# foollh/PicoPose

Measured on AMD Instinct MI355X. Metric: image-crops/sec (224x224, 162 templates), higher is better.
Workload: dtype f32 tensors; networks: f32 operands split into 2 f16 terms (22 bits) on f16 MFMA with f32 accumulate; stage-1 contraction: f16 MFMA operands, f32 accumulate, exact f32 re-evaluation of near-ties; PnP f64

## Files before the change

include/picopose_hip.h:

```cpp
#ifndef PICOPOSE_HIP_H
#define PICOPOSE_HIP_H

#include <stddef.h>
#include <stdint.h>

#ifdef __cplusplus
extern "C" {
#endif

#define PP_OK 0
#define PP_EINVAL (-1)
#define PP_EWORKSPACE (-2)
#define PP_ELAUNCH (-3)

#define PP_MATCH_EXACT 0
#define PP_MATCH_FAST 1

const char* pp_strerror(int code);
int pp_version(void);

int pp_prof_enable(int max_records);
int pp_prof_collect(float* out_ms, int max_out, int* count);
int pp_prof_gemm_enable(int max_records);
int pp_prof_gemm_collect(double* ms, double* flops, int* launches);
// ... 161 lines not shown
int pp_transpose_batched(const float* in, long long in_batch_stride, int B, int R, int C, float* out,
                         long long out_batch_stride, int ld_out, int col_off, void* stream);
int pp_assemble_tokens(const float* patches, const float* cls_token, const float* pos, int B, int T, int C,
                       float* tokens, void* stream);
int pp_normalize_rows(const float* x, int rows, int n, float eps, float* y, void* stream);

int pp_resize_bilinear_nhwc(const float* in, int B, int H, int W, int C, int Ho, int Wo, float mul,
                            float* out, void* stream);
int pp_resize_bilinear_nhwc_hl(const float* in, int B, int H, int W, int C, int Ho, int Wo, float mul, void* out_hl,
                               void* stream);
int pp_warp_nhwc(const float* feat, int feat_batch, const float* flow, int B, int H, int W, int C, int ld_flow,
                 float* out, int ld_out, void* stream);
int pp_warp_nhwc_hl(const float* feat, int feat_batch, const float* flow, int B, int H, int W, int C, int ld_flow,
                    void* out_hl, int ld_h, void* stream);
int pp_avgpool2_nhwc(const float* in, int B, int H, int W, int C, float* out, void* stream);
int pp_gather_rows(const float* src, const long long* index, long long n_src_rows, long long row_floats, int n, float* dst,
                   void* stream);
int pp_bank_rows_to_tokens(const float* bank, long long n_bank_rows, int C, int P, const long long* index, int n, float* tokens, int ld,
                           int T, int skip, void* stream);
int pp_patch_operand(const float* bank, long long n_bank_rows, const long long* index, int n, const float* front, int n_front, int H, int W,
                     void* out, int terms, void* stream);
int pp_flow_operand(const float* flow, int ld_flow, long long rows, void* out8, int terms, void* stream);

int pp_crop_resize_normalize(const unsigned char* image, int H, int W, const unsigned char* mask, int y1, int y2, int x1,
                             int x2, int S, int rgb_mask_flag, const double* mean3, const double* std3, float* out_rgb,
                             float* out_mask, void* stream);
int pp_depth_points_nearest(const float* depth_m, int H, int W, int y1, int y2, int x1, int x2, int P, float fx, float fy,
                            float cx, float cy, float* out_pts, void* stream);
int pp_corr_lookup_nhwc(const float* f1, int ld_f1, const float* f2_l0, const float* f2_l1, const float* f2_l2,
                        int f2_batch, const float* flow, int B, int H, int W, int C, int levels, int radius,
                        int ld_flow, float* out, int ld_out, void* stream);
int pp_corr_lookup_nhwc_ex(const float* f1, int ld_f1, const float* f2_l0, const float* f2_l1, const float* f2_l2,
                           int f2_batch, const float* flow, int B, int H, int W, int C, int levels, int radius,
                           int ld_flow, int prec, float* out, int ld_out, void* stream);

int pp_conv_narrow_hl(const void* x_hl, int ld_x, int B, int H, int W, int C, const float* weight, const float* bias, int ksize,
                      int n_out, const float* residual, float* out, void* stream);
int pp_conv_narrow_f32(const float* x, int ld_x, int B, int H, int W, int C, const float* weight, const float* bias, int ksize,
                       int n_out, const float* residual, float* out, void* stream);

int pp_winograd_input_f32(const float* x, int ld_x, long long batch_stride, int B, int H, int W, int C, int relu, float* U, void* stream);
int pp_winograd_weight_f32(const float* w, int Cout, int Cin, int ldw, float* V, void* stream);
int pp_winograd_output_f32(const float* Y, int B, int H, int W, int Cout, const float* bias, int act, const float* residual,
                           const float* residual2, float* out, int ldc, void* stream);

int pp_winograd4_input_hl(const void* x_hl, int ld_x, long long batch_stride, int B, int H, int W, int C, int relu, void* U_hl, long long P_pad,
                          void* stream);
int pp_winograd4_weight_f32(const float* w, int Cout, int Cin, int ldw, float* V, void* stream);
int pp_winograd4_output(const float* Y, int ld_y, int B, int H, int W, int Cout, const float* bias, int act, const float* residual,
                        const float* residual2, float* out, int ldc, void* out_hl, int ld_h, int c_relu, long long P_pad, void* stream);

int pp_winograd4_chain(const float* Y, int ld_y, int B, int H, int W, int C, const float* bias, int act, int c_relu, void* U_hl, long long P_pad,
                       void* stream);

int pp_winograd_chain_f32(const float* Y, int B, int H, int W, int C, const float* bias, int act, int relu_next, float* U, void* stream);

int pp_set_saturation_word(unsigned int* word);

int pp_saturation_take(unsigned int* word, unsigned int* slot, void* stream);


int pp_corr_lookup_nhwc_hl(const void* f1_hl, int ld_f1, const void* f2_hl_l0, const void* f2_hl_l1, const void* f2_hl_l2,
                           int f2_batch, const float* flow, int B, int H, int W, int C, int levels, int radius, int ld_flow,
                           float* out, int ld_out, void* stream);
int pp_corr_lookup_nhwc_hl_op(const void* f1_hl, int ld_f1, const void* f2_hl_l0, const void* f2_hl_l1, const void* f2_hl_l2,
                              int f2_batch, const float* flow, int B, int H, int W, int C, int levels, int radius, int ld_flow,
                              float* out, int ld_out, void* out_hl, int ld_out_h, void* stream);
int pp_avgpool2_hl(const float* in, int B, int H, int W, int C, float* out, void* out_hl, void* stream);

int pp_pnp_ransac(const float* tar_pts_2d, const float* src_pts_3d, const float* K, const float* tem_pose,
                  const int64_t* tar_pts, const int64_t* src_pts, int P, int H, int W, int N, int iterations,
                  float reproj_threshold, double* rot, double* tvec, double* inlier_ratio, int32_t* success,
                  int32_t* num_points, void* stream);

int pp_pnp_ransac_debug(const float* tar_pts_2d, const float* src_pts_3d, const float* K, const float* tem_pose,
                        const int64_t* tar_pts, const int64_t* src_pts, int P, int H, int W, int N, int iterations,
                        float reproj_threshold, double* rot, double* tvec, double* inlier_ratio, int32_t* success,
                        int32_t* num_points, double* refit_branches, void* stream);

int pp_pnp_ransac_refine(const float* tar_pts_2d, const float* src_pts_3d, const float* K, const float* tem_pose,
                         const int64_t* tar_pts, const int64_t* src_pts, int P, int H, int W, int N, int iterations,
                         float reproj_threshold, int max_iters, double eps, double* rot, double* tvec, double* inlier_ratio,
                         int32_t* success, int32_t* num_points, double* rms_before, double* rms_after, int32_t* lm_iterations,
                         uint8_t* inlier_mask, void* stream);

int pp_pnp_refine_lm(const double* object_points, const double* image_points, const int32_t* count, const double* K,
                     const double* rot_init, const double* tvec_init, int P, int Nmax, int max_iters, double eps, double* rot,
                     double* tvec, double* rms_before, double* rms_after, int32_t* lm_iterations, void* stream);

int pp_rgbd_ransac(const float* tar_pts_2d, const float* src_pts_3d, const float* K, const float* tem_pose,
                   const int64_t* tar_pts, const int64_t* src_pts, int P, int H, int W, int N,
                   const float* depth, int n_images, int dH, int dW, const int32_t* image_index,
                   const float* inlier_dist, int iterations,
                   double* rot, double* tvec, double* inlier_ratio, int32_t* success,
                   int32_t* num_points, int32_t* num_listed, double* rms, uint8_t* inlier_mask, void* stream);

size_t pp_train_keypoints_workspace_bytes(int B);
int pp_train_keypoints(const float* src_mask, const float* tar_mask, int mask_h, int mask_w, const float* src_depth,
                       const float* tar_depth, int depth_h, int depth_w, const float* src_Minv, const float* tar_Minv,
                       const float* src_M, const float* tar_M, const float* src_Kinv, const float* tar_Kinv, const float* src_K,
                       const float* tar_K, const float* T_src2tar, const float* T_tar2src, int B, float* src_pts, float* tar_pts,
                       void* workspace, size_t workspace_bytes, void* stream);
size_t pp_batchnorm_train_workspace_bytes(int rows, int C);
int pp_batchnorm_train(const float* x, const float* gamma, const float* beta, int rows, int C, float eps, float momentum,
                       float* running_mean, float* running_var, int relu, const float* residual, const float* residual2, float* y,
                       void* workspace, size_t workspace_bytes, void* stream);
// ... 236 lines not shown
```

picopose_amd/_lib.py:

```python
import ctypes
import os
import re

from .build import LIB

_HEADER = os.path.join(os.path.dirname(os.path.abspath(__file__)), "..", "include", "picopose_hip.h")

PP_OK = 0
PP_MATCH_EXACT = 0
PP_MATCH_FAST = 1
PP_BANK_F32 = 0
PP_BANK_F16 = 1

_lib = None


class PpGemmDesc(ctypes.Structure):
    _fields_ = [
        ("A", ctypes.c_void_p), ("B", ctypes.c_void_p), ("C", ctypes.c_void_p), ("bias", ctypes.c_void_p),
        ("gamma", ctypes.c_void_p), ("residual", ctypes.c_void_p), ("residual2", ctypes.c_void_p),
        ("M", ctypes.c_int), ("N", ctypes.c_int), ("K", ctypes.c_int),
        ("lda", ctypes.c_int), ("ldb", ctypes.c_int), ("ldc", ctypes.c_int), ("b_kn", ctypes.c_int),
        ("batch0", ctypes.c_int), ("batch1", ctypes.c_int),
        ("a_bs0", ctypes.c_longlong), ("a_bs1", ctypes.c_longlong), ("b_bs0", ctypes.c_longlong),
# ... 40 lines not shown
        if not os.path.exists(LIB):
            raise PicoPoseHipError(
                f"{LIB} not found: build it with `python -m picopose_amd.build` "
                "(hipcc --offload-arch=gfx950). There is no CPU fallback."
            )
        import torch

        L = ctypes.CDLL(LIB)
        c = ctypes
        vp, i32, f32, sz = c.c_void_p, c.c_int, c.c_float, c.c_size_t
        L.pp_strerror.restype = c.c_char_p
        L.pp_strerror.argtypes = [i32]
        L.pp_version.restype = i32
        L.pp_prof_enable.argtypes = [i32]
        L.pp_prof_collect.argtypes = [c.POINTER(f32), i32, c.POINTER(i32)]
        L.pp_prof_gemm_enable.argtypes = [i32]
        L.pp_prof_gemm_collect.argtypes = [c.POINTER(c.c_double), c.POINTER(c.c_double), c.POINTER(i32)]
        L.pp_prof_gemm_records.argtypes = [i32, c.POINTER(i32), c.POINTER(f32), c.POINTER(c.c_double), c.POINTER(i32)]
        L.pp_prof_gemm_records2.argtypes = [i32, c.POINTER(i32), c.POINTER(f32), c.POINTER(c.c_double), c.POINTER(c.c_double), c.POINTER(i32)]
        L.pp_gemm_tune_save.argtypes = [c.c_char_p]
        L.pp_gemm_tune_load.argtypes = [c.c_char_p]
        L.pp_gemm_tune_entries.argtypes = []
        L.pp_gemm_generic_epilogue.argtypes = [i32]
        L.pp_stage1_workspace_bytes.argtypes = [i32, i32, i32, c.POINTER(sz)]
        L.pp_stage1_scores.argtypes = [vp, vp, vp, i32, i32, i32, i32, i32, i32, f32, vp, sz, vp, vp, vp]
        L.pp_stage1_scores_ex.argtypes = [vp, i32, vp, vp, i32, i32, i32, i32, i32, i32, f32, vp, sz, vp, vp, vp]
        L.pp_topk.argtypes = [vp, i32, i32, i32, vp, vp, vp]
        L.pp_stage1_match.argtypes = [vp, vp, vp, i32, i32, i32, i32, i32, i32, i32, f32, vp, sz,
                                      vp, vp, vp, vp, vp]
        L.pp_stage1_match_ex.argtypes = [vp, i32, vp, vp, i32, i32, i32, i32, i32, i32, i32, f32, vp, sz, vp, vp, vp, vp, vp]
        L.pp_stage1_indexed_workspace_bytes.argtypes = [i32, i32, i32, c.POINTER(sz)]
        L.pp_stage1_scores_indexed.argtypes = [vp, i32, vp, i32, vp, vp, i32, i32, i32, i32, i32, i32, f32, vp, sz, vp, vp, vp]
        L.pp_stage1_match_indexed.argtypes = [vp, i32, vp, i32, vp, vp, i32, i32, i32, i32, i32, i32, i32, f32, vp, sz, vp, vp, vp,
                                              vp, vp]
        L.pp_similarity_volume.argtypes = [vp, vp, vp, i32, i32, i32, i32, vp, vp]
        L.pp_calc_pred_Ms.argtypes = [vp, vp, vp, vp, vp, vp, i32, f32, vp, vp]
        L.pp_pose_recovery_2d.argtypes = [vp, vp, vp, vp, vp, vp, i32, vp, vp]
        L.pp_init_correspondences.argtypes = [vp, vp, i32, i32, i32, vp, vp, vp]
        L.pp_stage3_correspondences.argtypes = [vp, vp, i32, i32, i32, f32, vp, vp, vp]
        L.pp_gather_valid.argtypes = [vp, vp, i32, i32, i32, i32, i32, vp, vp, vp]
        L.pp_gemm.argtypes = [c.POINTER(PpGemmDesc), vp]
        L.pp_split_f16x3.argtypes = [vp, c.c_longlong, vp, vp, vp]
        L.pp_split_activation.argtypes = [vp, c.c_longlong, i32, i32, i32, i32, i32, vp, vp]
        L.pp_split_activation_ld.argtypes = [vp, c.c_longlong, i32, i32, i32, i32, i32, vp, i32, vp]
        L.pp_conv_narrow_hl.argtypes = [vp, i32, i32, i32, i32, i32, vp, vp, i32, i32, vp, vp, vp]
        L.pp_conv_narrow_f32.argtypes = [vp, i32, i32, i32, i32, i32, vp, vp, i32, i32, vp, vp, vp]
        L.pp_winograd_input_f32.argtypes = [vp, i32, c.c_longlong, i32, i32, i32, i32, i32, vp, vp]
        L.pp_winograd_weight_f32.argtypes = [vp, i32, i32, i32, vp, vp]
        L.pp_winograd_output_f32.argtypes = [vp, i32, i32, i32, i32, vp, i32, vp, vp, vp, i32, vp]
        L.pp_winograd4_input_hl.argtypes = [vp, i32, c.c_longlong, i32, i32, i32, i32, i32, vp, c.c_longlong, vp]
        L.pp_winograd4_weight_f32.argtypes = [vp, i32, i32, i32, vp, vp]
        L.pp_winograd4_output.argtypes = [vp, i32, i32, i32, i32, i32, vp, i32, vp, vp, vp, i32, vp, i32, i32, c.c_longlong, vp]
        L.pp_winograd4_chain.argtypes = [vp, i32, i32, i32, i32, i32, vp, i32, i32, vp, c.c_longlong, vp]
        L.pp_winograd_chain_f32.argtypes = [vp, i32, i32, i32, i32, vp, i32, i32, vp, vp]
        L.pp_set_saturation_word.argtypes = [vp]
        L.pp_saturation_take.argtypes = [vp, vp, vp]
        L.pp_split_weights_t.argtypes = [vp, c.c_longlong, i32, vp, vp, vp]
        L.pp_split_weights_ws.argtypes = [vp, c.c_longlong, i32, vp, vp, vp, vp]
        L.pp_split_activation_t.argtypes = [vp, c.c_longlong, i32, i32, i32, i32, i32, vp, i32, i32, vp]
        L.pp_hl_patch_columns_t.argtypes = [vp, i32, i32, c.c_longlong, vp, i32, i32, i32, vp]
        L.pp_layernorm_t.argtypes = [vp, vp, vp, i32, i32, f32, vp, vp, i32, vp]
        L.pp_resize_bilinear_nhwc_t.argtypes = [vp, i32, i32, i32, i32, i32, i32, f32, vp, i32, vp]
        L.pp_resize_bilinear_nhwc_dual.argtypes = [vp, i32, i32, i32, i32, i32, i32, f32, vp, vp, i32, vp]
        L.pp_warp_nhwc_t.argtypes = [vp, i32, vp, i32, i32, i32, i32, i32, vp, i32, i32, vp]
        L.pp_attention_t.argtypes = [vp, i32, i32, i32, i32, i32, f32, vp, vp, vp]
        L.pp_sum_slices.argtypes = [vp, i32, i32, i32, vp, i32, vp, vp]
        L.pp_hl_patch_columns.argtypes = [vp, i32, i32, c.c_longlong, vp, i32, i32, vp]
        L.pp_warp_nhwc_hl.argtypes = [vp, i32, vp, i32, i32, i32, i32, i32, vp, i32, vp]
        L.pp_attention.argtypes = [vp, i32, i32, i32, i32, f32, vp, vp]
        L.pp_attention_split.argtypes = [vp, i32, i32, i32, i32, f32, vp, vp, vp]
        L.pp_attention_ex.argtypes = [vp, i32, i32, i32, i32, f32, i32, vp, vp, vp]
        L.pp_attention_hl.argtypes = [vp, i32, i32, i32, i32, f32, vp, vp, vp]
        L.pp_attention_train.argtypes = [vp, i32, i32, i32, i32, f32, vp, vp, vp]
        L.pp_attention_backward.argtypes = [vp, vp, vp, vp, vp, i32, i32, i32, i32, f32, vp, vp, vp]
        L.pp_layernorm.argtypes = [vp, vp, vp, i32, i32, f32, vp, vp]
        L.pp_layernorm_split.argtypes = [vp, vp, vp, i32, i32, f32, vp, vp, vp]
        L.pp_softmax_rows.argtypes = [vp, i32, i32, i32, vp]
        L.pp_groupnorm_nhwc.argtypes = [vp, vp, vp, i32, i32, i32, i32, f32, i32, vp, vp]
        L.pp_transpose_batched.argtypes = [vp, c.c_longlong, i32, i32, i32, vp, c.c_longlong, i32, i32, vp]
        L.pp_assemble_tokens.argtypes = [vp, vp, vp, i32, i32, i32, vp, vp]
        L.pp_normalize_rows.argtypes = [vp, i32, i32, f32, vp, vp]
        L.pp_resize_bilinear_nhwc.argtypes = [vp, i32, i32, i32, i32, i32, i32, f32, vp, vp]
        L.pp_resize_bilinear_nhwc_hl.argtypes = [vp, i32, i32, i32, i32, i32, i32, f32, vp, vp]
        L.pp_warp_nhwc.argtypes = [vp, i32, vp, i32, i32, i32, i32, i32, vp, i32, vp]
        L.pp_avgpool2_nhwc.argtypes = [vp, i32, i32, i32, i32, vp, vp]
        L.pp_gather_rows.argtypes = [vp, vp, c.c_longlong, c.c_longlong, i32, vp, vp]
        L.pp_bank_rows_to_tokens.argtypes = [vp, c.c_longlong, i32, i32, vp, i32, vp, i32, i32, i32, vp]
        L.pp_patch_operand.argtypes = [vp, c.c_longlong, vp, i32, vp, i32, i32, i32, vp, i32, vp]
        L.pp_flow_operand.argtypes = [vp, i32, c.c_longlong, vp, i32, vp]
        L.pp_depth_points_nearest.argtypes = [vp, i32, i32, i32, i32, i32, i32, i32, f32, f32, f32, f32, vp, vp]
        L.pp_crop_resize_normalize.argtypes = [vp, i32, i32, vp, i32, i32, i32, i32, i32, i32, c.POINTER(c.c_double),
                                               c.POINTER(c.c_double), vp, vp, vp]
        L.pp_corr_lookup_nhwc.argtypes = [vp, i32, vp, vp, vp, i32, vp, i32, i32, i32, i32, i32, i32, i32, vp, i32, vp]
        L.pp_corr_lookup_nhwc_ex.argtypes = [vp, i32, vp, vp, vp, i32, vp, i32, i32, i32, i32, i32, i32, i32, i32, vp, i32, vp]
        L.pp_corr_lookup_nhwc_hl.argtypes = [vp, i32, vp, vp, vp, i32, vp, i32, i32, i32, i32, i32, i32, i32, vp, i32, vp]
        L.pp_corr_lookup_nhwc_hl_op.argtypes = [vp, i32, vp, vp, vp, i32, vp, i32, i32, i32, i32, i32, i32, i32, vp, i32, vp, i32, vp]
        L.pp_avgpool2_hl.argtypes = [vp, i32, i32, i32, i32, vp, vp, vp]
        L.pp_pnp_ransac.argtypes = [vp, vp, vp, vp, vp, vp, i32, i32, i32, i32, i32, f32, vp, vp, vp, vp, vp, vp]
        L.pp_pnp_ransac_debug.argtypes = [vp, vp, vp, vp, vp, vp, i32, i32, i32, i32, i32, f32, vp, vp, vp, vp, vp, vp, vp]
        L.pp_pnp_ransac_refine.argtypes = [vp, vp, vp, vp, vp, vp, i32, i32, i32, i32, i32, f32, i32, c.c_double] + [vp] * 10
        L.pp_pnp_refine_lm.argtypes = [vp] * 6 + [i32, i32, i32, c.c_double] + [vp] * 6
        L.pp_rgbd_ransac.argtypes = [vp] * 6 + [i32] * 4 + [vp, i32, i32, i32, vp, vp, i32] + [vp] * 9
        L.pp_train_keypoints_workspace_bytes.restype = sz
        L.pp_train_keypoints_workspace_bytes.argtypes = [i32]
        L.pp_train_keypoints.argtypes = [vp, vp, i32, i32, vp, vp, i32, i32] + [vp] * 10 + [i32, vp, vp, vp, sz, vp]
        L.pp_batchnorm_train_workspace_bytes.restype = sz
# ... 113 lines not shown
```

picopose_amd/csrc/pp_winograd.hip:

```cpp
#include <hip/hip_runtime.h>
#include <stdint.h>
#include "../../include/picopose_hip.h"
#include "pp_common.h"

namespace {

typedef float f4 __attribute__((ext_vector_type(4)));

__device__ __forceinline__ void wino_bt_d_b(const f4 (&d)[4][4], f4 (&u)[4][4]) {
    f4 t[4][4];
#pragma unroll
    for (int c = 0; c < 4; ++c) {
        t[0][c] = d[0][c] - d[2][c];
        t[1][c] = d[1][c] + d[2][c];
        t[2][c] = d[2][c] - d[1][c];
        t[3][c] = d[1][c] - d[3][c];
    }
#pragma unroll
    for (int a = 0; a < 4; ++a) {
        u[a][0] = t[a][0] - t[a][2];
        u[a][1] = t[a][1] + t[a][2];
        u[a][2] = t[a][2] - t[a][1];
        u[a][3] = t[a][1] - t[a][3];
    }
// ... 410 lines not shown
                    wino_split4(x4, hi, lo, top);
#pragma unroll
                    for (int e = 0; e < 4; ++e) f[e] = (float)hi[e] + (float)lo[e];
                    *(f4*)(slot + ((oy * W) + 4 * tx + ox) * CHN_PX + 4 * q) = f;
                }
            }
        }
        if (half >= 1 && live && r >= 2) {
            constexpr int RPG = 6 / NB;
            const int R = r - 2, a0 = NB == 2 ? RPG * (half - 1) : 0;
            f4 t[6][6];
#pragma unroll
            for (int dx = 0; dx < 6; ++dx) {
                f4 d[6];
                const int px = 4 * tx - 1 + dx;
#pragma unroll
                for (int dy = 0; dy < 6; ++dy) {
                    const int g = 4 * R - 1 + dy;
                    const int gc = min(max(g, 0), H - 1), pc = min(max(px, 0), W - 1);
                    f4 v = *(const f4*)(chs + ((gc >> 2) & 3) * SLOT + ((gc & 3) * W + pc) * CHN_PX + 4 * q);
                    if (!(g >= 0 && g < H && px >= 0 && px < W)) v = f4{0.f, 0.f, 0.f, 0.f};
                    d[dy] = v;
                }
                PP_W4_BT(d[0], d[1], d[2], d[3], d[4], d[5], t[0][dx], t[1][dx], t[2][dx], t[3][dx], t[4][dx], t[5][dx])
            }
            const long long p = ((long long)b * th + R) * TW + tx;
            const unsigned uoff = (unsigned)((p * 2 * C + gcol + par * 8) * 2);
#pragma unroll
            for (int ai = 0; ai < RPG; ++ai) {
                f4 u[6];
                if constexpr (NB == 2) {
                    f4 t0 = t[ai][0], t1 = t[ai][1], t2 = t[ai][2], t3 = t[ai][3], t4 = t[ai][4], t5 = t[ai][5];
                    if (a0) {
                        t0 = t[3 + ai][0], t1 = t[3 + ai][1], t2 = t[3 + ai][2];
                        t3 = t[3 + ai][3], t4 = t[3 + ai][4], t5 = t[3 + ai][5];
                    }
                    PP_W4_BT(t0, t1, t2, t3, t4, t5, u[0], u[1], u[2], u[3], u[4], u[5])
                } else {
                    PP_W4_BT(t[ai][0], t[ai][1], t[ai][2], t[ai][3], t[ai][4], t[ai][5], u[0], u[1], u[2], u[3], u[4], u[5])
                }
#pragma unroll
                for (int bb = 0; bb < 6; ++bb) {
                    hf4 hi, lo;
                    wino_split4(u[bb] * (1.f / 64.f), hi, lo, top);
                    __builtin_amdgcn_raw_buffer_store_b128(wino_pair_pack(par, hi, lo), wino_block_rsrc(U, wino_opaque(6 * (a0 + ai) + bb), blk), uoff, 0, PP_WINO_ST_AUX);
                }
            }
        }
        __syncthreads();
    }
    wino_note_sat(!(top < 65504.f), sat);
}

template <int W>
__global__ __launch_bounds__(2 * (W / 2) * 8, 4) void wino2_chain_kernel(const float* __restrict__ Y, int H, int C, long long P, const float* __restrict__ bias,
                                                                       int act, int relu_next, float* __restrict__ U) {
    constexpr int TW = W / 2, NI = TW * 8;
    constexpr int SLOT = 2 * W * CHN_PX;
    extern __shared__ __attribute__((aligned(16))) float chs[];
    const int th = H >> 1, nsl = C >> 5;
    const int b = blockIdx.x / nsl, cs = blockIdx.x - b * nsl;
    const int half = threadIdx.x / NI, it = threadIdx.x - half * NI, tx = it >> 3, q = it & 7;
    const int c = cs * 32 + 4 * q;
    const f4 bv = bias ? *(const f4*)(bias + c) : f4{0.f, 0.f, 0.f, 0.f};
    for (int r = 0; r < th + 2; ++r) {
        if (half == 0 && r < th) {
            const long long p = ((long long)b * th + r) * TW + tx;
            f4 y[4][4];
#pragma unroll
            for (int a = 0; a < 4; ++a)
#pragma unroll
                for (int bb = 0; bb < 4; ++bb) y[a][bb] = *(const f4*)(Y + ((long long)(4 * a + bb) * P + p) * C + c);
            float* slot = chs + (r & 3) * SLOT;
#pragma unroll
            for (int oy = 0; oy < 2; ++oy)
#pragma unroll
                for (int ox = 0; ox < 2; ++ox) {
                    f4 col[4], o;
#pragma unroll
                    for (int bb = 0; bb < 4; ++bb) col[bb] = oy == 0 ? (y[0][bb] + y[1][bb]) + y[2][bb] : (y[1][bb] - y[2][bb]) - y[3][bb];
                    o = ox == 0 ? (col[0] + col[1]) + col[2] : (col[1] - col[2]) - col[3];
#pragma unroll
                    for (int e = 0; e < 4; ++e) {
                        float v = wino_act(o[e] + bv[e], act);
                        o[e] = relu_next ? (v > 0.f ? v : 0.f) : v;
                    }
                    *(f4*)(slot + (oy * W + 2 * tx + ox) * CHN_PX + 4 * q) = o;
                }
        }
        if (half == 1 && r >= 2) {
            const int R = r - 2;
            f4 t[4][4];
#pragma unroll
            for (int dx = 0; dx < 4; ++dx) {
                f4 d[4];
#pragma unroll
                for (int dy = 0; dy < 4; ++dy) {
                    const int g = 2 * R - 1 + dy, px = 2 * tx - 1 + dx;
                    const int gc = min(max(g, 0), H - 1), pc = min(max(px, 0), W - 1);
                    f4 v = *(const f4*)(chs + ((gc >> 1) & 3) * SLOT + ((gc & 1) * W + pc) * CHN_PX + 4 * q);
                    if (!(g >= 0 && g < H && px >= 0 && px < W)) v = f4{0.f, 0.f, 0.f, 0.f};
                    d[dy] = v;
                }
                t[0][dx] = d[0] - d[2];
                t[1][dx] = d[1] + d[2];
                t[2][dx] = d[2] - d[1];
                t[3][dx] = d[1] - d[3];
            }
            const long long p = ((long long)b * th + R) * TW + tx;
#pragma unroll
            for (int a = 0; a < 4; ++a) {
                const f4 u0 = t[a][0] - t[a][2], u1 = t[a][1] + t[a][2], u2 = t[a][2] - t[a][1], u3 = t[a][1] - t[a][3];
                *(f4*)(U + ((long long)(4 * a + 0) * P + p) * C + c) = u0;
                *(f4*)(U + ((long long)(4 * a + 1) * P + p) * C + c) = u1;
                *(f4*)(U + ((long long)(4 * a + 2) * P + p) * C + c) = u2;
                *(f4*)(U + ((long long)(4 * a + 3) * P + p) * C + c) = u3;
            }
        }
        __syncthreads();
    }
}

template <int W>
static int wino2_chain_launch(const float* Y, int B, int H, int C, const float* bias, int act, int relu_next, float* U, hipStream_t st) {
    constexpr int threads = 2 * (W / 2) * 8;
    const size_t lds = (size_t)4 * 2 * W * CHN_PX * sizeof(float);
    static signed char attr[PP_MAX_DEVICES];
    signed char& ok = attr[pp_cur_device()];
    if (ok == 0)
        ok = hipFuncSetAttribute((const void*)wino2_chain_kernel<W>, hipFuncAttributeMaxDynamicSharedMemorySize, (int)lds) == hipSuccess ? 1 : -1;
    if (ok < 0) return PP_ELAUNCH;
    const long long P = (long long)B * (H / 2) * (W / 2);
    hipLaunchKernelGGL(wino2_chain_kernel<W>, dim3((unsigned)(B * (C / 32))), dim3(threads), lds, st, Y, H, C, P, bias, act, relu_next, U);
    return pp_last_launch();
}

template <int W>
static int wino4_chain_launch(const float* Y, int B, int H, int C, const float* bias, int act, int c_relu, void* U, long long Pp, int ldy, hipStream_t st) {
    constexpr int NB = W == 64 ? 2 : 1;
    constexpr int threads = (1 + NB) * ((W / 4) * 8 < 64 ? 64 : (W / 4) * 8);
    const size_t lds = (size_t)4 * 4 * W * CHN_PX * sizeof(float);
    static signed char attr[PP_MAX_DEVICES];
    signed char& ok = attr[pp_cur_device()];
    if (ok == 0)
        ok = hipFuncSetAttribute((const void*)wino4_chain_kernel<W, NB>, hipFuncAttributeMaxDynamicSharedMemorySize, (int)lds) == hipSuccess ? 1 : -1;
    if (ok < 0) return PP_ELAUNCH;
    hipLaunchKernelGGL((wino4_chain_kernel<W, NB>), dim3((unsigned)(B * (C / 32))), dim3(threads), lds, st, Y, H, C, bias, act, c_relu, (_Float16*)U, Pp,
                       ldy, pp_saturation_word());
    return pp_last_launch();
}

static inline int grid8_of(long long n) {
    const long long g = ((n + 255) / 256 + 7) / 8 * 8;
    return (int)g;
}

static inline int grid_of(long long n) {
    const long long g = (n + 255) / 256;
    return (int)(g < 1 ? 1 : (g > 65535 * 8 ? 65535 * 8 : g));
}

}

extern "C" {

int pp_winograd_input_f32(const float* x, int ld_x, long long batch_stride, int B, int H, int W, int C, int relu, float* U, void* stream) {
    if (!x || !U || B <= 0 || H < 2 || W < 2 || (H & 1) || (W & 1) || C <= 0 || (C & 3) || ld_x < C || (ld_x & 3) || (batch_stride & 3)) return PP_EINVAL;
    if (((uintptr_t)x & 15) || ((uintptr_t)U & 15)) return PP_EINVAL;
    const long long total = (long long)B * (H / 2) * (W / 2) * (C / 4);
    hipLaunchKernelGGL(wino_input_kernel, dim3(grid_of(total)), dim3(256), 0, (hipStream_t)stream, x, ld_x, batch_stride, B, H, W, C, relu, U);
    return pp_last_launch();
}

int pp_winograd_weight_f32(const float* w, int Cout, int Cin, int ldw, float* V, void* stream) {
    if (!w || !V || Cout <= 0 || Cin <= 0 || ldw < 9 * Cin) return PP_EINVAL;
    hipLaunchKernelGGL(wino_weight_kernel, dim3(grid_of((long long)Cout * Cin)), dim3(256), 0, (hipStream_t)stream, w, Cout, Cin, ldw, V);
    return pp_last_launch();
}

int pp_winograd_output_f32(const float* Y, int B, int H, int W, int Cout, const float* bias, int act, const float* residual,
                           const float* residual2, float* out, int ldc, void* stream) {
    if (!Y || !out || B <= 0 || H < 2 || W < 2 || (H & 1) || (W & 1) || Cout <= 0 || ldc < Cout) return PP_EINVAL;
    if (act != PP_ACT_NONE && act != PP_ACT_RELU && act != PP_ACT_LEAKY01) return PP_EINVAL;
    const bool vec = (Cout & 3) == 0 && (ldc & 3) == 0 && (((uintptr_t)Y | (uintptr_t)out | (uintptr_t)residual | (uintptr_t)residual2 | (uintptr_t)bias) & 15) == 0;
    const long long total = (long long)B * (H / 2) * (W / 2) * (vec ? Cout / 4 : Cout);
    if (vec)
        hipLaunchKernelGGL(wino_output_kernel<true>, dim3(grid_of(total)), dim3(256), 0, (hipStream_t)stream, Y, B, H, W, Cout, bias, act, residual,
                           residual2, out, ldc);
    else
        hipLaunchKernelGGL(wino_output_kernel<false>, dim3(grid_of(total)), dim3(256), 0, (hipStream_t)stream, Y, B, H, W, Cout, bias, act, residual,
                           residual2, out, ldc);
    return pp_last_launch();
}


int pp_winograd4_input_hl(const void* x_hl, int ld_x, long long batch_stride, int B, int H, int W, int C, int relu, void* U_hl, long long P_pad,
                          void* stream) {
    if (!x_hl || !U_hl || B <= 0 || H < 4 || W < 4 || (H & 3) || (W & 3) || C <= 0 || (C & 7) || ld_x < C || (ld_x & 7) || (batch_stride & 7)) return PP_EINVAL;
    if (((uintptr_t)x_hl & 15) || ((uintptr_t)U_hl & 15)) return PP_EINVAL;
    const long long total = (long long)B * (H / 4) * (W / 4) * (C / 4);
    if ((total + 255) / 256 + 8 >= (1LL << 31) || P_pad < (long long)B * (H / 4) * (W / 4)) return PP_EINVAL;
    const long long x_bytes = ((long long)(B - 1) * batch_stride + (long long)(H * W - 1) * ld_x + C) * 4;
    if (x_bytes + (long long)(W + 1) * ld_x * 4 >= 0xFFFFFF00LL || P_pad * C * 4 >= 0xFFFFFF00LL) return PP_EINVAL;
    if (relu)
        hipLaunchKernelGGL(wino4_input_kernel<true>, dim3(grid8_of(total)), dim3(256), 0, (hipStream_t)stream, (const _Float16*)x_hl, (unsigned)x_bytes,
                           ld_x, batch_stride, B, H, W, C, (_Float16*)U_hl, P_pad, pp_saturation_word());
    else
        hipLaunchKernelGGL(wino4_input_kernel<false>, dim3(grid8_of(total)), dim3(256), 0, (hipStream_t)stream, (const _Float16*)x_hl, (unsigned)x_bytes,
                           ld_x, batch_stride, B, H, W, C, (_Float16*)U_hl, P_pad, pp_saturation_word());
    return pp_last_launch();
}

int pp_winograd4_weight_f32(const float* w, int Cout, int Cin, int ldw, float* V, void* stream) {
    if (!w || !V || Cout <= 0 || Cin <= 0 || ldw < 9 * Cin) return PP_EINVAL;
    const long long total = (long long)Cout * Cin;
    hipLaunchKernelGGL(wino4_weight_kernel, dim3((unsigned)((total + 255) / 256)), dim3(256), 0, (hipStream_t)stream, w, Cout, Cin, ldw, V);
    return pp_last_launch();
}

int pp_winograd4_output(const float* Y, int ld_y, int B, int H, int W, int Cout, const float* bias, int act, const float* residual,
                        const float* residual2, float* out, int ldc, void* out_hl, int ld_h, int c_relu, long long P_pad, void* stream) {
    if (P_pad < (long long)B * (H / 4) * (W / 4) || ld_y < Cout || (ld_y & 3) || P_pad * ld_y * 4 >= 0xFFFFFF00LL) return PP_EINVAL;
    if (!Y || (!out && !out_hl) || B <= 0 || H < 4 || W < 4 || (H & 3) || (W & 3) || Cout <= 0 || (Cout & 3)) return PP_EINVAL;
    if (act != PP_ACT_NONE && act != PP_ACT_RELU && act != PP_ACT_LEAKY01) return PP_EINVAL;
    if (out && (ldc < Cout || (ldc & 3))) return PP_EINVAL;
    if (!out && (residual || residual2)) return PP_EINVAL;
    if (out_hl && ((Cout & 7) || ld_h < Cout || (ld_h & 7))) return PP_EINVAL;
    if (((uintptr_t)Y | (uintptr_t)out | (uintptr_t)residual | (uintptr_t)residual2 | (uintptr_t)bias | (uintptr_t)out_hl) & 15) return PP_EINVAL;
    const long long total = (long long)B * (H / 4) * (W / 4) * (Cout / 4);
    if ((total + 255) / 256 + 8 >= (1LL << 31)) return PP_EINVAL;
    hipLaunchKernelGGL(wino4_output_kernel, dim3(grid8_of(total)), dim3(256), 0, (hipStream_t)stream, Y, B, H, W, Cout, bias, act, residual, residual2,
                       out, ldc, (_Float16*)out_hl, ld_h, c_relu, P_pad, ld_y, pp_saturation_word());
    return pp_last_launch();
}


int pp_winograd4_chain(const float* Y, int ld_y, int B, int H, int W, int C, const float* bias, int act, int c_relu, void* U_hl, long long P_pad,
                       void* stream) {
    if (!Y || !U_hl || B <= 0 || H < 4 || (H & 3) || (W != 16 && W != 32 && W != 64) || C <= 0 || (C & 31) || ld_y < C || (ld_y & 3)) return PP_EINVAL;
    if (P_pad * ld_y * 4 >= 0xFFFFFF00LL) return PP_EINVAL;
    if (act != PP_ACT_NONE && act != PP_ACT_RELU && act != PP_ACT_LEAKY01) return PP_EINVAL;
    if (P_pad < (long long)B * (H / 4) * (W / 4) || P_pad * C * 4 >= 0xFFFFFF00LL || (long long)B * (C / 32) >= (1LL << 31)) return PP_EINVAL;
    if (((uintptr_t)Y | (uintptr_t)U_hl | (uintptr_t)bias) & 15) return PP_EINVAL;
    hipStream_t st = (hipStream_t)stream;
    if (W == 64) return wino4_chain_launch<64>(Y, B, H, C, bias, act, c_relu, U_hl, P_pad, ld_y, st);
    if (W == 32) return wino4_chain_launch<32>(Y, B, H, C, bias, act, c_relu, U_hl, P_pad, ld_y, st);
    return wino4_chain_launch<16>(Y, B, H, C, bias, act, c_relu, U_hl, P_pad, ld_y, st);
}


int pp_winograd_chain_f32(const float* Y, int B, int H, int W, int C, const float* bias, int act, int relu_next, float* U, void* stream) {
    if (!Y || !U || B <= 0 || H < 2 || (H & 1) || (W != 16 && W != 32 && W != 64) || C <= 0 || (C & 31)) return PP_EINVAL;
    if (act != PP_ACT_NONE && act != PP_ACT_RELU && act != PP_ACT_LEAKY01) return PP_EINVAL;
    if ((long long)B * (C / 32) >= (1LL << 31) || (((uintptr_t)Y | (uintptr_t)U | (uintptr_t)bias) & 15)) return PP_EINVAL;
    hipStream_t st = (hipStream_t)stream;
    if (W == 64) return wino2_chain_launch<64>(Y, B, H, C, bias, act, relu_next, U, st);
    if (W == 32) return wino2_chain_launch<32>(Y, B, H, C, bias, act, relu_next, U, st);
    return wino2_chain_launch<16>(Y, B, H, C, bias, act, relu_next, U, st);
}

}
```

picopose_amd/ops.py:

```python
import contextlib
import ctypes
import os
import threading

import torch

from . import _lib
from ._lib import PpGemmDesc

ACT = {None: 0, "none": 0, "relu": 1, "gelu": 2, "leaky01": 3, "tanh": 4}

PRECISION = "f16x3"
_PREC = {"f32": 0, "f16x3": 1, "f16": 2}
_split_cache = {}
_scope = threading.local()


def precision():
    return getattr(_scope, "mode", None) or PRECISION


def check_precision(mode):
    if mode is not None and mode not in _PREC:
        raise ValueError(f"unknown arithmetic mode {mode!r}: expected None or one of {sorted(_PREC)}")
# ... 707 lines not shown
               "pp_winograd_output_f32")
    return out


WINOGRAD4 = os.environ.get("PP_WINOGRAD4", "1") != "0"
WINO4_GROUPS_PER_LAUNCH = 36
WINO4_U_SCALE = 1.0 / 16.0


class WinoInput4:
    __slots__ = ("U", "geom", "src")

    def __init__(self, U, geom, src):
        self.U, self.geom, self.src = U, geom, src


def _winograd4_ok(B, H, W, cin, cout):
    P = B * (H // 4) * (W // 4)
    return (precision() == "f16x3" and WINOGRAD4 and H % 4 == 0 and W % 4 == 0 and cin % 8 == 0 and cout % 8 == 0
            and 36 * (P + 255) < 2 ** 31 and not torch.is_grad_enabled())


def _wino4_rows(P):
    return -(-P // 256) * 256


def winograd4_weight(wp, cin):
    key = (wp.data_ptr(), tuple(wp.shape), "wino4")
    hit = _wino_cache.get(key)
    if hit is None or hit[2] != wp._version:
        Cout = wp.shape[0]
        V = hit[0] if hit is not None else torch.empty(36 * Cout, cin, dtype=torch.float32, device=wp.device)
        hl = hit[3] if hit is not None else torch.empty(36 * Cout, 2 * cin, dtype=torch.float16, device=wp.device)
        _lib.check(_lib.lib().pp_winograd4_weight_f32(_p(wp), Cout, cin, wp.shape[1], _p(V), _lib.stream_ptr()), "pp_winograd4_weight_f32")
        scale = torch.empty(1, dtype=torch.float32, device=wp.device)
        _lib.check(_lib.lib().pp_split_weights_t(_p(V), V.numel(), 2, _p(hl), _p(scale), _lib.stream_ptr()), "pp_split_weights_t")
        if len(_wino_cache) > 1024:
            _wino_cache.clear()
        hit = _wino_cache[key] = (V, wp, wp._version, hl, float(scale.item()))
    return hit[0], hit[3], hit[4]


def _winograd4_input(src_ptr, ld_x, B, H, W, cin, dev):
    P = B * (H // 4) * (W // 4)
    Pp = _wino4_rows(P)
    U = Split((torch.empty if Pp == P else torch.zeros)(36 * Pp, 2 * cin, dtype=torch.float16, device=dev), 2)
    _lib.check(_lib.lib().pp_winograd4_input_hl(src_ptr, ld_x, H * W * ld_x, B, H, W, cin, 0, _p(U.hl), Pp, _lib.stream_ptr()), "pp_winograd4_input_hl")
    _chk(U.hl, "pp_winograd4_input_hl")
    return U


WINO4_CHAIN = os.environ.get("PP_WINOGRAD4_CHAIN", "1") != "0"
WINO4_CHAIN_WIDTHS = (32, 64)


def _wino4_products(U, V, vhl, vscale, Pp, cin, N):
    Y = torch.empty(36, Pp, N, dtype=torch.float32, device=U.device)
    per = max(1, min(WINO4_GROUPS_PER_LAUNCH, 0xF0000000 // (4 * Pp * max(cin, N))))
    for x0 in range(0, 36, per):
        n = min(per, 36 - x0)
        _run(_desc(A_hl=U.hl.data_ptr() + x0 * Pp * cin * 4, B=_p(V), B_hl=vhl.data_ptr() + x0 * N * cin * 4, b_scale=vscale, C=_p(Y[x0]),
                   M=Pp, N=N, K=cin, lda=cin, ldb=cin, ldc=N, prec=_PREC["f16x3"], batch0=n, a_bs0=Pp * cin, b_bs0=N * cin,
                   c_bs0=Pp * N, alpha=PP_A_SCALE / WINO4_U_SCALE, _keep=(U, vhl, V)))
    return Y


def _wino4_finish(Y, col0, ldy, bias, B, H, W, Cout, act, residual, residual2, out, out_split, split_relu, also_split, chain_next):
    P = B * (H // 4) * (W // 4)
    Pp, dev, L = _wino4_rows(P), Y.device, _lib.lib()
    yp = Y.data_ptr() + 4 * col0
    ret, hl_t, ldc = None, None, 0
    if (chain_next and WINO4_CHAIN and out_split and out is None and residual is None and residual2 is None and W in WINO4_CHAIN_WIDTHS and Cout % 32 == 0
            and _winograd4_ok(B, H, W, Cout, Cout)):
        U1 = Split((torch.empty if Pp == P else torch.zeros)(36 * Pp, 2 * Cout, dtype=torch.float16, device=dev), 2)
        _lib.check(L.pp_winograd4_chain(yp, ldy, B, H, W, Cout, _p(bias), ACT[act], int(split_relu), _p(U1.hl), Pp, _lib.stream_ptr()), "pp_winograd4_chain")
        _chk(U1.hl, "pp_winograd4_chain")
        return WinoInput4(U1, (B, H, W, Cout), None)
    if out_split and out is None and residual is None and residual2 is None:
        hl_t = Split.empty(B * H * W, Cout, dev)
        hl_t.image = (B, H, W)
        ret, c_relu = hl_t, int(split_relu)
    else:
        if out is None:
            out = torch.empty(B, H, W, Cout, dtype=torch.float32, device=dev)
        ldc = out.stride(2)
        assert out.stride(3) == 1 and out.stride(1) == W * ldc and out.stride(0) == H * W * ldc
        for r_ in (residual, residual2):
            if r_ is not None:
                assert r_.stride() == out.stride()
        ret, c_relu = out, 0
        if also_split is not None and out.is_contiguous():
            hl_t = Split.empty(B * H * W, Cout, dev)
            hl_t.image = (B, H, W)
            c_relu = int(also_split == "relu")
            setattr(out, "_hl_relu" if also_split == "relu" else "_hl", hl_t)
    _lib.check(L.pp_winograd4_output(yp, ldy, B, H, W, Cout, _p(bias), ACT[act], _p(residual), _p(residual2), _p(out), ldc,
                                     _p(hl_t.hl) if hl_t is not None else None, Cout, c_relu, Pp, _lib.stream_ptr()), "pp_winograd4_output")
    if hl_t is not None:
        _chk(hl_t.hl, "pp_winograd4_output")
    return ret


def _conv3x3_winograd4(x, wp, bias, B, H, W, cin, Cout, act, residual, residual2, out, out_split, split_relu, also_split, chain_next=False):
    P = B * (H // 4) * (W // 4)
    V, vhl, vscale = winograd4_weight(wp, cin)
    if isinstance(x, WinoInput4):
        assert x.geom == (B, H, W, cin)
        U = x.U
    elif isinstance(x, tuple):
        U = _winograd4_input(x[0].col_ptr(x[1]), x[0].shape[1], B, H, W, cin, x[0].device)
    else:
        U = _winograd4_input(x.hl.data_ptr(), x.shape[1], B, H, W, cin, x.device)
    Pp = _wino4_rows(P)
    assert U.hl.shape[0] == 36 * Pp
    Y = _wino4_products(U, V, vhl, vscale, Pp, cin, Cout)
    return _wino4_finish(Y, 0, Cout, bias, B, H, W, Cout, act, residual, residual2, out, out_split, split_relu, also_split, chain_next)


WINO4_PAIR = os.environ.get("PP_WINOGRAD4_PAIR", "1") != "0"


def winograd4_weight_pair(wp_a, wp_b, cin):
    key = (wp_a.data_ptr(), wp_b.data_ptr(), tuple(wp_a.shape), tuple(wp_b.shape), "wino4pair")
    hit = _wino_cache.get(key)
    if hit is None or hit[2] != (wp_a._version, wp_b._version):
        Va, Vb = winograd4_weight(wp_a, cin)[0], winograd4_weight(wp_b, cin)[0]
        Ca, Cb = wp_a.shape[0], wp_b.shape[0]
        V = torch.cat([Va.view(36, Ca, cin), Vb.view(36, Cb, cin)], dim=1).reshape(36 * (Ca + Cb), cin).contiguous()
# ... 335 lines not shown
```

Measured before the change: 582.9.

## Add persistent warp-specialized walking kernel for Winograd-4 output-to-input chain

Adds a persistent Winograd F(4,3) chain kernel. A producer wave group does the output transform, bias, activation and split-rounding for one tile row and writes it into a 4-slot LDS ring. One or two consumer groups read rows from that ring, apply the next layer's input transform and store the f16 hi/lo U tiles. Each block walks a contiguous range of (batch, channel-slice) items down the image, so overlapping tile rows are reused from LDS instead of recomputed or reloaded. The grid is capped at resident capacity. This is enabled by default through an env flag and adds a per-row __syncthreads plus a large dynamic-LDS footprint.

```diff
diff --git a/include/picopose_hip.h b/include/picopose_hip.h
--- a/include/picopose_hip.h
+++ b/include/picopose_hip.h
@@ -237,6 +237,8 @@
 
 int pp_winograd4_chain(const float* Y, int ld_y, int B, int H, int W, int C, const float* bias, int act, int c_relu, void* U_hl, long long P_pad,
                        void* stream);
+int pp_winograd4_chain_v(const float* Y, int ld_y, int B, int H, int W, int C, const float* bias, int act, int c_relu, void* U_hl, long long P_pad,
+                         int groups, void* stream);
 
 int pp_winograd_chain_f32(const float* Y, int B, int H, int W, int C, const float* bias, int act, int relu_next, float* U, void* stream);
 
diff --git a/picopose_amd/_lib.py b/picopose_amd/_lib.py
--- a/picopose_amd/_lib.py
+++ b/picopose_amd/_lib.py
@@ -116,6 +116,7 @@
         L.pp_winograd4_weight_f32.argtypes = [vp, i32, i32, i32, vp, vp]
         L.pp_winograd4_output.argtypes = [vp, i32, i32, i32, i32, i32, vp, i32, vp, vp, vp, i32, vp, i32, i32, c.c_longlong, vp]
         L.pp_winograd4_chain.argtypes = [vp, i32, i32, i32, i32, i32, vp, i32, i32, vp, c.c_longlong, vp]
+        L.pp_winograd4_chain_v.argtypes = [vp, i32, i32, i32, i32, i32, vp, i32, i32, vp, c.c_longlong, i32, vp]
         L.pp_winograd_chain_f32.argtypes = [vp, i32, i32, i32, i32, vp, i32, i32, vp, vp]
         L.pp_set_saturation_word.argtypes = [vp]
         L.pp_saturation_take.argtypes = [vp, vp, vp]
diff --git a/picopose_amd/csrc/pp_winograd.hip b/picopose_amd/csrc/pp_winograd.hip
--- a/picopose_amd/csrc/pp_winograd.hip
+++ b/picopose_amd/csrc/pp_winograd.hip
@@ -486,6 +486,132 @@
     wino_note_sat(!(top < 65504.f), sat);
 }
 
+template <int V>
+struct wino_int {
+    static constexpr int value = V;
+};
+
+template <int W, int NB>
+__global__ __launch_bounds__((1 + NB) * ((W / 4) * 8 < 64 ? 64 : (W / 4) * 8)) void wino4_chain_walk_kernel(const float* __restrict__ Y, int H, int C, int nitems,
+                                                                            const float* __restrict__ bias, int act, int c_relu, _Float16* __restrict__ U,
+                                                                            long long Pp, int ldy, unsigned* sat) {
+    constexpr int TW = W / 4, NI = TW * 8;
+    constexpr int GS = NI < 64 ? 64 : NI;
+    constexpr int SLOT = 4 * W * CHN_PX;
+    extern __shared__ __attribute__((aligned(16))) float chs[];
+    const int th = H >> 2, nsl = C >> 5;
+    const unsigned G = gridDim.x;
+    const unsigned lw = (G & 7) ? blockIdx.x : (blockIdx.x & 7) * (G >> 3) + (blockIdx.x >> 3);
+    const int i0 = (int)((long long)lw * nitems / G), i1 = (int)((long long)(lw + 1) * nitems / G);
+    const int nrows = (i1 - i0) * th;
+    const int grp = __builtin_amdgcn_readfirstlane((int)threadIdx.x / GS);
+    const int it = (int)threadIdx.x - grp * GS, tx = it >> 3, q = it & 7;
+    const bool live = NI >= GS || it < NI;
+    const unsigned long long blk = (unsigned long long)Pp * C * 4, blky = (unsigned long long)Pp * ldy * 4;
+    const int par = q & 1;
+    float top = 0.f;
+    if (grp == 0) {
+        const float slope = act == PP_ACT_RELU ? 0.f : (act == PP_ACT_LEAKY01 ? 0.1f : 1.f);
+        const float hfloor = c_relu ? 0.f : -INFINITY;
+        auto y_off = [&](int v, int& c) -> unsigned {
+            const int item = i0 + v / th, r = v - (v / th) * th;
+            const int b = item / nsl, cs = item - b * nsl;
+            c = cs * 32 + 4 * q;
+            const long long p = ((long long)b * th + r) * TW + tx;
+            return (live && v < nrows) ? (unsigned)((p * ldy + c) * 4) : 0xFFFFFFFFu;
+        };
+        f4 y[6][6], bv = {0.f, 0.f, 0.f, 0.f};
+        {
+            int c;
+            const unsigned yoff = y_off(0, c);
+#pragma unroll
+            for (int bb = 0; bb < 6; ++bb)
+#pragma unroll
+                for (int a = 0; a < 6; ++a)
+                    y[a][bb] = __builtin_bit_cast(f4, __builtin_amdgcn_raw_buffer_load_b128(wino_block_rsrc(Y, wino_opaque(6 * a + bb), blky), yoff, 0, PP_WINO_LD_AUX));
+            if (bias) bv = *(const f4*)(bias + c);
+        }
+        for (int k = 0; k < nrows + 2; ++k) {
+            if (k < nrows) {
+                f4 z[4][6];
+#pragma unroll
+                for (int bb = 0; bb < 6; ++bb) PP_W4_AT(y[0][bb], y[1][bb], y[2][bb], y[3][bb], y[4][bb], y[5][bb], z[0][bb], z[1][bb], z[2][bb], z[3][bb])
+                const f4 bvk = bv;
+                int cn;
+                const unsigned yoff = y_off(k + 1, cn);
+                float* slot = chs + (k & 3) * SLOT;
+#pragma unroll
+                for (int oy = 0; oy < 4; ++oy) {
+                    f4 o[4];
+                    PP_W4_AT(z[oy][0], z[oy][1], z[oy][2], z[oy][3], z[oy][4], z[oy][5], o[0], o[1], o[2], o[3])
+#pragma unroll
+                    for (int ox = 0; ox < 4; ++ox) {
+                        f4 v = o[ox] + bvk, x4, f;
+#pragma unroll
+                        for (int e = 0; e < 4; ++e) {
+                            v[e] = fmaxf(v[e], v[e] * slope);
+                            x4[e] = fmaxf(v[e] * PP_A_SCALE, hfloor);
+                        }
+                        hf4 hi, lo;
+                        wino_split4(x4, hi, lo, top);
+#pragma unroll
+                        for (int e = 0; e < 4; ++e) f[e] = (float)hi[e] + (float)lo[e];
+                        *(f4*)(slot + ((oy * W) + 4 * tx + ox) * CHN_PX + 4 * q) = f;
+                    }
+#pragma unroll
+                    for (int n = 9 * oy; n < 9 * oy + 9; ++n)
+                        y[n % 6][n / 6] = __builtin_bit_cast(f4, __builtin_amdgcn_raw_buffer_load_b128(wino_block_rsrc(Y, wino_opaque(6 * (n % 6) + n / 6), blky), yoff, 0, PP_WINO_LD_AUX));
+                }
+                if (bias && k + 1 < nrows) bv = *(const f4*)(bias + cn);
+            }
+            __syncthreads();
+        }
+    } else {
+        for (int k = 0; k < nrows + 2; ++k) {
+            if (live && k >= 2) {
+                const int v = k - 2, j = v / th, R = v - j * th, v0 = v - R;
+                const int item = i0 + j, b = item / nsl, cs = item - b * nsl;
+                const int c = cs * 32 + 4 * q, gcol = (c >> 3) << 4;
+                f4 t[6][6];
+#pragma unroll
+                for (int dx = 0; dx < 6; ++dx) {
+                    f4 d[6];
+                    const int px = 4 * tx - 1 + dx;
+#pragma unroll
+                    for (int dy = 0; dy < 6; ++dy) {
+                        const int g = 4 * R - 1 + dy;
+                        const int gc = min(max(g, 0), H - 1), pc = min(max(px, 0), W - 1);
+                        const unsigned m = (unsigned)wino_opaque(__builtin_amdgcn_readfirstlane(g >= 0 && g < H ? -1 : 0)) & (px >= 0 && px < W ? ~0u : 0u);
+                        const wu4 vv = *(const wu4*)(chs + ((v0 + (gc >> 2)) & 3) * SLOT + ((gc & 3) * W + pc) * CHN_PX + 4 * q);
+                        d[dy] = __builtin_bit_cast(f4, vv & m);
+                    }
+                    PP_W4_BT(d[0], d[1], d[2], d[3], d[4], d[5], t[0][dx], t[1][dx], t[2][dx], t[3][dx], t[4][dx], t[5][dx])
+                }
+                const long long p = ((long long)b * th + R) * TW + tx;
+                const unsigned uoff = (unsigned)((p * 2 * C + gcol + par * 8) * 2);
+                auto rows = [&](auto a0c) {
+                    constexpr int a0 = decltype(a0c)::value;
+#pragma unroll
+                    for (int a = a0; a < a0 + 6 / NB; ++a) {
+                        f4 u[6];
+                        PP_W4_BT(t[a][0], t[a][1], t[a][2], t[a][3], t[a][4], t[a][5], u[0], u[1], u[2], u[3], u[4], u[5])
+#pragma unroll
+                        for (int bb = 0; bb < 6; ++bb) {
+                            hf4 hi, lo;
+                            wino_split4(u[bb] * (1.f / 64.f), hi, lo, top);
+                            __builtin_amdgcn_raw_buffer_store_b128(wino_pair_pack(par, hi, lo), wino_block_rsrc(U, wino_opaque(6 * a + bb), blk), uoff, 0, PP_WINO_ST_AUX);
+                        }
+                    }
+                };
+                if (NB == 1 || grp == 1) rows(wino_int<0>{});
+                else rows(wino_int<3>{});
+            }
+            __syncthreads();
+        }
+    }
+    wino_note_sat(!(top < 65504.f), sat);
+}
+
 template <int W>
 __global__ __launch_bounds__(2 * (W / 2) * 8, 4) void wino2_chain_kernel(const float* __restrict__ Y, int H, int C, long long P, const float* __restrict__ bias,
                                                                        int act, int relu_next, float* __restrict__ U) {
@@ -584,6 +710,25 @@
     return pp_last_launch();
 }
 
+template <int W>
+static int wino4_chain_walk_launch(const float* Y, int B, int H, int C, const float* bias, int act, int c_relu, void* U, long long Pp, int ldy, int groups,
+                                   hipStream_t st) {
+    constexpr int NB = W == 64 ? 2 : 1;
+    constexpr int threads = (1 + NB) * ((W / 4) * 8 < 64 ? 64 : (W / 4) * 8);
+    const size_t lds = (size_t)4 * 4 * W * CHN_PX * sizeof(float);
+    static signed char attr[PP_MAX_DEVICES];
+    signed char& ok = attr[pp_cur_device()];
+    if (ok == 0)
+        ok = hipFuncSetAttribute((const void*)wino4_chain_walk_kernel<W, NB>, hipFuncAttributeMaxDynamicSharedMemorySize, (int)lds) == hipSuccess ? 1 : -1;
+    if (ok < 0) return PP_ELAUNCH;
+    const long long items = (long long)B * (C / 32), resident = (long long)pp_cu_count() * (64 / W);
+    long long grid = items < resident ? items : resident;
+    if (groups > 0 && groups < grid) grid = groups;
+    hipLaunchKernelGGL((wino4_chain_walk_kernel<W, NB>), dim3((unsigned)grid), dim3(threads), lds, st, Y, H, C, (int)items, bias, act, c_relu, (_Float16*)U,
+                       Pp, ldy, pp_saturation_word());
+    return pp_last_launch();
+}
+
 static inline int grid8_of(long long n) {
     const long long g = ((n + 255) / 256 + 7) / 8 * 8;
     return (int)g;
@@ -671,12 +816,22 @@
 
 int pp_winograd4_chain(const float* Y, int ld_y, int B, int H, int W, int C, const float* bias, int act, int c_relu, void* U_hl, long long P_pad,
                        void* stream) {
+    return pp_winograd4_chain_v(Y, ld_y, B, H, W, C, bias, act, c_relu, U_hl, P_pad, -1, stream);
+}
+
+int pp_winograd4_chain_v(const float* Y, int ld_y, int B, int H, int W, int C, const float* bias, int act, int c_relu, void* U_hl, long long P_pad,
+                         int groups, void* stream) {
     if (!Y || !U_hl || B <= 0 || H < 4 || (H & 3) || (W != 16 && W != 32 && W != 64) || C <= 0 || (C & 31) || ld_y < C || (ld_y & 3)) return PP_EINVAL;
     if (P_pad * ld_y * 4 >= 0xFFFFFF00LL) return PP_EINVAL;
     if (act != PP_ACT_NONE && act != PP_ACT_RELU && act != PP_ACT_LEAKY01) return PP_EINVAL;
     if (P_pad < (long long)B * (H / 4) * (W / 4) || P_pad * C * 4 >= 0xFFFFFF00LL || (long long)B * (C / 32) >= (1LL << 31)) return PP_EINVAL;
     if (((uintptr_t)Y | (uintptr_t)U_hl | (uintptr_t)bias) & 15) return PP_EINVAL;
     hipStream_t st = (hipStream_t)stream;
+    if (groups) {
+        if (W == 64) return wino4_chain_walk_launch<64>(Y, B, H, C, bias, act, c_relu, U_hl, P_pad, ld_y, groups, st);
+        if (W == 32) return wino4_chain_walk_launch<32>(Y, B, H, C, bias, act, c_relu, U_hl, P_pad, ld_y, groups, st);
+        return wino4_chain_walk_launch<16>(Y, B, H, C, bias, act, c_relu, U_hl, P_pad, ld_y, groups, st);
+    }
     if (W == 64) return wino4_chain_launch<64>(Y, B, H, C, bias, act, c_relu, U_hl, P_pad, ld_y, st);
     if (W == 32) return wino4_chain_launch<32>(Y, B, H, C, bias, act, c_relu, U_hl, P_pad, ld_y, st);
     return wino4_chain_launch<16>(Y, B, H, C, bias, act, c_relu, U_hl, P_pad, ld_y, st);
diff --git a/picopose_amd/ops.py b/picopose_amd/ops.py
--- a/picopose_amd/ops.py
+++ b/picopose_amd/ops.py
@@ -783,6 +783,7 @@
 
 WINO4_CHAIN = os.environ.get("PP_WINOGRAD4_CHAIN", "1") != "0"
 WINO4_CHAIN_WIDTHS = (32, 64)
+WINO4_CHAIN_WALK = os.environ.get("PP_WINOGRAD4_CHAIN_WALK", "1") != "0"
 
 
 def _wino4_products(U, V, vhl, vscale, Pp, cin, N):
@@ -804,7 +805,8 @@
     if (chain_next and WINO4_CHAIN and out_split and out is None and residual is None and residual2 is None and W in WINO4_CHAIN_WIDTHS and Cout % 32 == 0
             and _winograd4_ok(B, H, W, Cout, Cout)):
         U1 = Split((torch.empty if Pp == P else torch.zeros)(36 * Pp, 2 * Cout, dtype=torch.float16, device=dev), 2)
-        _lib.check(L.pp_winograd4_chain(yp, ldy, B, H, W, Cout, _p(bias), ACT[act], int(split_relu), _p(U1.hl), Pp, _lib.stream_ptr()), "pp_winograd4_chain")
+        _lib.check(L.pp_winograd4_chain_v(yp, ldy, B, H, W, Cout, _p(bias), ACT[act], int(split_relu), _p(U1.hl), Pp, -1 if WINO4_CHAIN_WALK else 0,
+                                          _lib.stream_ptr()), "pp_winograd4_chain")
         _chk(U1.hl, "pp_winograd4_chain")
         return WinoInput4(U1, (B, H, W, Cout), None)
     if out_split and out is None and residual is None and residual2 is None:
```

New measurement: 586.9, median of 6. Within noise of the previous version (+0.7%).
